# ChrisTho23/DrakeGPT

Measured on AMD Instinct MI355X. Metric: training tokens/sec (fwd+bwd+AdamW), higher is better.
Workload: dtype bf16; 1 GPU; TransformerLM_scaled: V=80 C=384 T=256 heads=6 layers=6 dropout=0.2; fwd+bwd+AdamW; hipGraph=on; batch_per_gpu=64, global_batch=64, seq_len=256, parallelism=dp1, dp_gradient_buckets=1, params=10800464

## Files before the change

### drakegpt_amd/csrc/chain.hip

```cpp
#include "common.h"
#include <stdlib.h>

typedef __attribute__((address_space(1))) const void* gptr_t;
typedef __attribute__((address_space(3))) void* lptr_t;

#define CH_C 384
#define CH_ROWS 64
#define CH_STAGE_B 24576
#define CH_STAGE_A 4096
#define CH_STAGE (CH_STAGE_B + CH_STAGE_A)
#define CH_NST 4
#define CH_ARES (CH_NST * CH_STAGE)
#define CH_KS (CH_C / 32)

struct ChainP {
    const char* o;
    const float* x;
    const char* wproj; const float* bproj;
    float* x1;
    const float* ln2w; const float* ln2b; float* mean2; float* rstd2; bf16_t* h2;
    const char* w1; const float* b1; bf16_t* f; unsigned char* bits;
    const char* w2; const float* b2;
    float* x2; bf16_t* x2b;
    const float* ln1w; const float* ln1b; float* mean1; float* rstd1; bf16_t* h1;
// ... 482 lines not shown
            }
        }
        stamp(12);
        if (HAS_QKV) {
            for (int c = 0; c < 3; ++c) {
                piece(KS, false, c < 2, MODE == 0 && c == 0);
                stamp(13 + 2 * c);
                if (p.dbg == 4 || p.dbg == 5) continue;
                const int lo = opaque_lane(), fr = lo & 15, fg = lo >> 4, col_l = wn * 96 + (fg & 1) * 16 + (fg >> 1) * 8;
#pragma unroll
                for (int q = 0; q < 3; ++q) {
                    const int col = c * C + col_l + 32 * q;
#pragma unroll
                    for (int i = 0; i < 2; ++i) {
                        const int64_t row = row0 + wm * 32 + i * 16 + fr;
                        float v[8];
                        take(i, q, v);
                        bf16x8 o;
#pragma unroll
                        for (int e = 0; e < 8; ++e) o[e] = (bf16_t)v[e];
                        if (p.dbg != 6) *(bf16x8*)(p.qkv + row0 * (3 * C) + mad24(wm * 32 + i * 16 + fr, 3 * C, col)) = o;
                    }
                }
                stamp(14 + 2 * c);
            }
        }
        stamp(19);
        __builtin_amdgcn_s_barrier();
        stamp(20);
    }
}

struct PackOne { const unsigned short* src; unsigned short* dst; int N, K; int64_t ld; };
__global__ __launch_bounds__(256) void pack_chain_kernel(const int64_t* __restrict__ desc, int n_desc, PackOne one) {
    const unsigned short* src = one.src;
    unsigned short* dst = one.dst;
    int K = one.K;
    int64_t ld = one.ld;
    int k = blockIdx.x;
    if (desc) {
        int d = 0;
        for (int i = 1; i < n_desc; ++i)
            if ((int64_t)blockIdx.x >= desc[i * 6 + 4]) d = i;
        const int64_t* D = desc + d * 6;
        src = (const unsigned short*)D[0]; dst = (unsigned short*)D[1]; K = (int)D[3]; ld = D[5];
        k = (int)((int64_t)blockIdx.x - D[4]);
    }
    const int KT = K / 32, c = k / KT, t = k % KT;
    if (!(KT & 1)) {
        const int half = t & 1, t0 = t - half;
        const int64_t k0 = k - half;
#pragma unroll
        for (int u = 0; u < 6; ++u) {
            const int idx = threadIdx.x + 256 * u, line = 96 * half + (idx >> 4), hi = (idx >> 3) & 1, j = idx & 7;
            const int slot = (hi * 4 + (j & 3)) ^ (line & 7);
            const int row = c * 384 + line + 192 * hi, col = t0 * 32 + 8 * j;
            *(u32x4*)(dst + ((k0 + (j >> 2)) * 1536 + line * 8 + slot) * 8) = *(const u32x4*)(src + (int64_t)row * ld + col);
        }
        return;
    }
#pragma unroll
    for (int u = 0; u < 6; ++u) {
        const int idx = threadIdx.x + 256 * u, line = idx >> 3, slot = idx & 7, ls = slot ^ (line & 7);
        const int row = c * 384 + line + 192 * (ls >> 2), col = t * 32 + 8 * (ls & 3);
        *(u32x4*)(dst + ((int64_t)k * 1536 + idx) * 8) = *(const u32x4*)(src + (int64_t)row * ld + col);
    }
}

extern "C" int dg_pack_chain_weights(const void* w, int64_t ld, void* packed, int N, int K, void* stream) {
    if (!w || !packed || N <= 0 || K <= 0 || N % 384 || K % 32 || ld < K || ld % 8 || !dg_aligned16(w) || !dg_aligned16(packed)) return DG_ERR_ARG;
    PackOne one{(const unsigned short*)w, (unsigned short*)packed, N, K, ld};
    hipLaunchKernelGGL(pack_chain_kernel, dim3((N / 384) * (K / 32)), dim3(256), 0, (hipStream_t)stream, (const int64_t*)nullptr, 0, one);
    DG_LAUNCH_CHECK();
    return DG_OK;
}

extern "C" int dg_pack_chain_weights_batched(const int64_t* desc, int n_desc, int total_stages, void* stream) {
    if (!desc || n_desc <= 0 || total_stages <= 0) return DG_ERR_ARG;
    PackOne one{nullptr, nullptr, 0, 0, 0};
    hipLaunchKernelGGL(pack_chain_kernel, dim3(total_stages), dim3(256), 0, (hipStream_t)stream, desc, n_desc, one);
    DG_LAUNCH_CHECK();
    return DG_OK;
}

__global__ __launch_bounds__(256) void l2_warm_kernel(const char* __restrict__ p, int64_t n_lines, float* __restrict__ sink) {
    const int j = (int)blockIdx.x >> 3, per = (int)gridDim.x >> 3;
    float acc = 0.f;
    for (int64_t i = (int64_t)j * 256 + threadIdx.x; i < n_lines; i += (int64_t)per * 256) acc += *(const float*)(p + i * 128);
    if (acc == 123.456f && sink) sink[0] = acc;
}

extern "C" int dg_l2_warm(const void* p, int64_t bytes, void* stream) {
    if (!p || bytes <= 0 || (((uintptr_t)p) & 127)) return DG_ERR_ARG;
    hipLaunchKernelGGL(l2_warm_kernel, dim3(256), dim3(256), 0, (hipStream_t)stream, (const char*)p, bytes / 128, (float*)nullptr);
    DG_LAUNCH_CHECK();
    return DG_OK;
}

static int ch_num_cus() {
    static const int v = [] {
        int dev = 0, n = 256;
        if (hipGetDevice(&dev) == hipSuccess) {
            int x = 0;
            if (hipDeviceGetAttribute(&x, hipDeviceAttributeMultiprocessorCount, dev) == hipSuccess && x > 0) n = x;
        }
        return n;
    }();
    return v;
}

extern "C" int dg_block_chain_supported(int M, int C) { return M > 0 && M % CH_ROWS == 0 && C == CH_C; }

static unsigned long long* g_chain_stamps = nullptr;
// ... 45 lines not shown
```

### drakegpt_amd/csrc/elementwise.hip

```cpp
#include "common.h"

__global__ void state_advance_kernel(uint32_t* st) { st[2] += 1u; }

extern "C" int dg_state_advance(uint32_t* rng_state, void* stream) {
    if (!rng_state) return DG_ERR_ARG;
    hipLaunchKernelGGL(state_advance_kernel, dim3(1), dim3(1), 0, (hipStream_t)stream, rng_state);
    DG_LAUNCH_CHECK();
    return DG_OK;
}

__global__ void batch_gather_kernel(const int64_t* __restrict__ corpus, int64_t n_corpus,
                                    const int64_t* __restrict__ off, int64_t* __restrict__ x,
                                    int64_t* __restrict__ y, int B, int T) {
    int64_t i = (int64_t)blockIdx.x * blockDim.x + threadIdx.x;
    if (i >= (int64_t)B * T) return;
    int b = (int)(i / T), t = (int)(i % T);
    int64_t o = off[b] + t;
    int64_t o1 = o + 1;
    if (o < 0) o = 0; if (o >= n_corpus) o = n_corpus - 1;
    if (o1 < 0) o1 = 0; if (o1 >= n_corpus) o1 = n_corpus - 1;
    x[i] = corpus[o];
    y[i] = corpus[o1];
}

extern "C" int dg_batch_gather(const int64_t* corpus, int64_t n_corpus, const int64_t* offsets,
                               int64_t* x, int64_t* y, int B, int T, void* stream) {
    if (!corpus || !offsets || !x || !y || B <= 0 || T <= 0 || n_corpus < 2) return DG_ERR_ARG;
    int64_t n = (int64_t)B * T;
    hipLaunchKernelGGL(batch_gather_kernel, dim3((unsigned)((n + 255) / 256)), dim3(256), 0,
                       (hipStream_t)stream, corpus, n_corpus, offsets, x, y, B, T);
    DG_LAUNCH_CHECK();
    return DG_OK;
}

struct BatchSrc {
    const int64_t* corpus; int64_t n_corpus; const int64_t* offsets; const uint32_t* step_state; const uint32_t* ctl;
    int64_t* x_ids; int64_t* y_ids; int B;
};
template <int VEC, bool GATHER = false>
__global__ void embed_fwd_kernel(const int64_t* __restrict__ idx, const float* __restrict__ tok,
                                 const float* __restrict__ pos, float* __restrict__ x,
                                 int64_t M, int T, int C, int V, bf16_t* __restrict__ onehot, int64_t ld_onehot, BatchSrc bs) {
    const int cv = C / VEC;
    int64_t total = M * cv;
    const int64_t* off = nullptr;
    if (GATHER) {
        uint32_t row = 0;
        if (bs.ctl) {
            const uint32_t n_rows = bs.ctl[1];
            row = bs.step_state[2] - bs.ctl[0];
            if (row >= n_rows) row = n_rows ? n_rows - 1 : 0;
        }
        off = bs.offsets + (int64_t)row * bs.B;
    }
    (void)total;
    const int lane = threadIdx.x & 63;
    const int64_t wave0 = ((int64_t)blockIdx.x * blockDim.x + threadIdx.x) >> 6, nwaves = ((int64_t)gridDim.x * blockDim.x) >> 6;
    for (int64_t m = wave0; m < M; m += nwaves) {
        const uint32_t mu = (uint32_t)__builtin_amdgcn_readfirstlane((int)m);
        const uint32_t bq = mu / (uint32_t)T;
        const int t = (int)(mu - bq * (uint32_t)T);
        int64_t v;
        if (GATHER) {
            int64_t o = off[bq] + t, o1 = o + 1;
            if (o < 0) o = 0; if (o >= bs.n_corpus) o = bs.n_corpus - 1;
            if (o1 < 0) o1 = 0; if (o1 >= bs.n_corpus) o1 = bs.n_corpus - 1;
            v = bs.corpus[o];
            if (lane == 0) { bs.x_ids[m] = v; bs.y_ids[m] = bs.corpus[o1]; }
        } else {
            v = idx[m];
        }
        v = v < 0 ? 0 : (v >= V ? V - 1 : v);
      for (int j = lane; j < cv; j += 64) {
        const int c = j * VEC;
        if (onehot) {
            if (VEC == 4 && j * 8 < ld_onehot) {
                bf16x8 o;
#pragma unroll
                for (int e = 0; e < 8; ++e) o[e] = (bf16_t)((int64_t)(j * 8 + e) == v ? 1.f : 0.f);
                *(bf16x8*)(onehot + m * ld_onehot + j * 8) = o;
            }
        }
        if (VEC == 4) {
            f32x4 a = *(const f32x4*)(tok + v * C + c);
            if (pos) a += *(const f32x4*)(pos + (int64_t)t * C + c);
            *(f32x4*)(x + m * C + c) = a;
        } else {
            float a = tok[v * C + c];
            if (pos) a += pos[(int64_t)t * C + c];
            x[m * C + c] = a;
        }
      }
    }
}

extern "C" int dg_embed_fwd(const int64_t* idx, const float* tok, const float* pos, float* x,
                            int B, int T, int C, int V, void* onehot, int64_t ld_onehot, void* stream) {
    if (!idx || !tok || !x || B <= 0 || T <= 0 || C <= 0 || V <= 0) return DG_ERR_ARG;
    if (onehot && (C % 4 || ld_onehot % 8 || ld_onehot < V || (int64_t)(C / 4) * 8 < ld_onehot || !dg_aligned16(onehot))) return DG_ERR_ARG;
    int64_t M = (int64_t)B * T;
    bool vec = (C % 4 == 0) && dg_aligned16(tok) && dg_aligned16(x) && (!pos || dg_aligned16(pos));
    int64_t total = vec ? M * (C / 4) : M * C;
    unsigned grid = (unsigned)((total + 255) / 256);
    if (grid > 4096) grid = 4096;
    if (vec)
        hipLaunchKernelGGL(embed_fwd_kernel<4>, dim3(grid), dim3(256), 0, (hipStream_t)stream, idx, tok, pos, x, M, T, C, V, (bf16_t*)onehot, ld_onehot, BatchSrc{});
    else {
        if (onehot) return DG_ERR_ALIGN;
        hipLaunchKernelGGL(embed_fwd_kernel<1>, dim3(grid), dim3(256), 0, (hipStream_t)stream, idx, tok, pos, x, M, T, C, V, (bf16_t*)nullptr, (int64_t)0, BatchSrc{});
    }
    DG_LAUNCH_CHECK();
    return DG_OK;
}

extern "C" int dg_batch_embed_fwd(const int64_t* corpus, int64_t n_corpus, const int64_t* offsets, const uint32_t* step_state,
                                  const uint32_t* ctl, int64_t* x_ids, int64_t* y_ids, const float* tok, const float* pos, float* x,
                                  int B, int T, int C, int V, void* onehot, int64_t ld_onehot, void* stream) {
    if (!corpus || !offsets || !x_ids || !y_ids || !tok || !x || B <= 0 || T <= 0 || C <= 0 || V <= 0 || n_corpus < 2) return DG_ERR_ARG;
    if ((ctl != nullptr) != (step_state != nullptr)) return DG_ERR_ARG;
    if (onehot && (C % 4 || ld_onehot % 8 || ld_onehot < V || (int64_t)(C / 4) * 8 < ld_onehot || !dg_aligned16(onehot))) return DG_ERR_ARG;
    int64_t M = (int64_t)B * T;
    bool vec = (C % 4 == 0) && dg_aligned16(tok) && dg_aligned16(x) && (!pos || dg_aligned16(pos));
    int64_t total = vec ? M * (C / 4) : M * C;
    unsigned grid = (unsigned)((total + 255) / 256);
    if (grid > 4096) grid = 4096;
    const BatchSrc bs{corpus, n_corpus, offsets, step_state, ctl, x_ids, y_ids, B};
    if (vec)
        hipLaunchKernelGGL((embed_fwd_kernel<4, true>), dim3(grid), dim3(256), 0, (hipStream_t)stream, (const int64_t*)nullptr, tok, pos, x, M, T, C, V, (bf16_t*)onehot, ld_onehot, bs);
    else {
        if (onehot) return DG_ERR_ALIGN;
        hipLaunchKernelGGL((embed_fwd_kernel<1, true>), dim3(grid), dim3(256), 0, (hipStream_t)stream, (const int64_t*)nullptr, tok, pos, x, M, T, C, V, (bf16_t*)nullptr, (int64_t)0, bs);
    }
    DG_LAUNCH_CHECK();
    return DG_OK;
}

__global__ void embed_window_kernel(const int64_t* __restrict__ ids, int64_t ld_ids, const uint32_t* __restrict__ state,
                                    const float* __restrict__ tok, const float* __restrict__ pos, float* __restrict__ x,
                                    int B, int Tw, int C, int V, int mode) {
    const int64_t L = (int64_t)state[2];
    if (L < 1 || L > ld_ids || (mode == 0 ? L > Tw : L < Tw)) return;
    const int rows_per_b = mode == 0 ? 1 : Tw;
    const int lane = threadIdx.x & 63;
    const int64_t wave0 = ((int64_t)blockIdx.x * blockDim.x + threadIdx.x) >> 6, nwaves = ((int64_t)gridDim.x * blockDim.x) >> 6;
    const int64_t Mrows = (int64_t)B * rows_per_b;
    for (int64_t m = wave0; m < Mrows; m += nwaves) {
        const int b = (int)(m / rows_per_b), i = (int)(m % rows_per_b);
        const int64_t col = mode == 0 ? L - 1 : L - Tw + i;
        const int t = mode == 0 ? (int)(L - 1) : i;
        int64_t v = ids[(int64_t)b * ld_ids + col];
        v = v < 0 ? 0 : (v >= V ? V - 1 : v);
        for (int c = lane; c < C; c += 64) x[m * C + c] = tok[v * C + c] + pos[(int64_t)t * C + c];
    }
}

extern "C" int dg_embed_window(const int64_t* ids, int64_t ld_ids, const uint32_t* state, const float* tok, const float* pos,
                               float* x, int B, int Tw, int C, int V, int mode, void* stream) {
    if (!ids || !state || !tok || !pos || !x || ld_ids <= 0 || B <= 0 || Tw <= 0 || C <= 0 || V <= 0 || (mode != 0 && mode != 1))
// ... 8 lines not shown

__global__ void zero_f32_kernel(float* __restrict__ p, int64_t n) {
    const int64_t n4 = n / 4;
    for (int64_t i = (int64_t)blockIdx.x * blockDim.x + threadIdx.x; i < n4; i += (int64_t)gridDim.x * blockDim.x)
        ((f32x4*)p)[i] = (f32x4){0.f, 0.f, 0.f, 0.f};
    for (int64_t i = n4 * 4 + (int64_t)blockIdx.x * blockDim.x + threadIdx.x; i < n; i += (int64_t)gridDim.x * blockDim.x) p[i] = 0.f;
}

template <typename TX>
__global__ void embed_bwd_tok_kernel(const int64_t* __restrict__ idx, const TX* __restrict__ dx,
                                     float* __restrict__ dtok, int64_t M, int C, int V) {
    int64_t total = M * C;
    for (int64_t i = (int64_t)blockIdx.x * blockDim.x + threadIdx.x; i < total;
         i += (int64_t)gridDim.x * blockDim.x) {
        int64_t m = i / C;
        int c = (int)(i % C);
        int64_t v = idx[m];
        v = v < 0 ? 0 : (v >= V ? V - 1 : v);
        atomicAdd(dtok + v * C + c, (float)dx[i]);
    }
}
template <typename TX>
__global__ __launch_bounds__(256) void embed_bwd_pos_kernel(const TX* __restrict__ dx, float* __restrict__ dpos,
                                                            int B, int T, int C) {
    __shared__ f32x4 red[4][64];
    const int64_t tc = (int64_t)T * C;
    const int lane = threadIdx.x & 63, g = threadIdx.x >> 6;
    const int64_t i = ((int64_t)blockIdx.x * 64 + lane) * 4;
    const bool vec = (tc % 4 == 0);
    f32x4 s = {0.f, 0.f, 0.f, 0.f};
    if (i < tc) {
        if (vec) {
            typedef TX TX4 __attribute__((ext_vector_type(4)));
            for (int b = g; b < B; b += 4) {
                const TX4 t = *(const TX4*)(dx + (int64_t)b * tc + i);
                s += (f32x4){(float)t[0], (float)t[1], (float)t[2], (float)t[3]};
            }
        } else {
            for (int b = g; b < B; b += 4)
#pragma unroll
                for (int e = 0; e < 4; ++e)
                    if (i + e < tc) s[e] += (float)dx[(int64_t)b * tc + i + e];
        }
    }
    red[g][lane] = s;
    __syncthreads();
    if (g == 0 && i < tc) {
        const f32x4 t = (red[0][lane] + red[1][lane]) + (red[2][lane] + red[3][lane]);
#pragma unroll
        for (int e = 0; e < 4; ++e)
            if (i + e < tc) dpos[i + e] = t[e];
    }
}
extern "C" int dg_embed_bwd(const int64_t* idx, const void* dx_v, int dx_dtype, float* dtok, float* dpos,
                            int B, int T, int C, int V, void* stream) {
    if (dx_dtype != DG_F32 && dx_dtype != DG_BF16) return DG_ERR_DTYPE;
    const float* dx = (const float*)dx_v;
    if (!idx || !dx || (!dtok && !dpos) || B <= 0 || T <= 0 || C <= 0 || V <= 0) return DG_ERR_ARG;
    hipStream_t s = (hipStream_t)stream;
    int64_t M = (int64_t)B * T;
    if (dtok) {
        const int64_t nz = (int64_t)V * C;
        if (!dg_aligned16(dtok)) return DG_ERR_ALIGN;
        unsigned zgrid = (unsigned)((nz / 4 + 255) / 256);
        if (zgrid < 1) zgrid = 1; if (zgrid > 4096) zgrid = 4096;
        hipLaunchKernelGGL(zero_f32_kernel, dim3(zgrid), dim3(256), 0, s, dtok, nz);
        DG_LAUNCH_CHECK();
        int64_t total = M * C;
// ... 74 lines not shown
    else if (dtype == DG_F32)
        hipLaunchKernelGGL(transpose_cast_kernel<float>, grid, dim3(256), 0, (hipStream_t)stream, in, ldi, (float*)out, ldo, R, Cc);
    else
        return DG_ERR_DTYPE;
    DG_LAUNCH_CHECK();
    return DG_OK;
}

template <typename TI, typename TO>
__global__ void transpose_cast_batched_kernel(const int64_t* __restrict__ desc, int n_desc) {
    __shared__ float tile[64][65];
    int d = 0;
    for (int i = 1; i < n_desc; ++i)
        if ((int64_t)blockIdx.x >= desc[i * 8 + 6]) d = i;
    const int64_t* D = desc + d * 8;
    const TI* in = (const TI*)D[0];
    TO* out = (TO*)D[1];
    const int64_t ldi = D[2], ldo = D[3];
    const int R = (int)D[4], Cc = (int)D[5];
    const int local = (int)((int64_t)blockIdx.x - D[6]), tiles_x = (int)D[7];
    const int r0 = (local / tiles_x) * 64, c0 = (local % tiles_x) * 64;
    const int tx = threadIdx.x & 63, ty = threadIdx.x >> 6;
    for (int i = ty; i < 64; i += 4) {
        int r = r0 + i, c = c0 + tx;
        tile[i][tx] = (r < R && c < Cc) ? to_f32<TI>(in[(int64_t)r * ldi + c]) : 0.f;
    }
    __syncthreads();
    for (int i = ty; i < 64; i += 4) {
        int c = c0 + i, r = r0 + tx;
        if (c < Cc && r < ldo) out[(int64_t)c * ldo + r] = from_f32<TO>(tile[tx][i]);
    }
}

__global__ __launch_bounds__(256) void transpose_bf16_batched_kernel(const int64_t* __restrict__ desc, int n_desc) {
    constexpr int PITCH = 68;
    __shared__ __attribute__((aligned(16))) unsigned short tile[64 * PITCH];
    int d = 0;
    for (int i = 1; i < n_desc; ++i)
        if ((int64_t)blockIdx.x >= desc[i * 8 + 6]) d = i;
    const int64_t* D = desc + d * 8;
    const unsigned short* in = (const unsigned short*)D[0];
    unsigned short* out = (unsigned short*)D[1];
    const int64_t ldi = D[2], ldo = D[3];
    const int R = (int)D[4], Cc = (int)D[5];
    const int local = (int)((int64_t)blockIdx.x - D[6]), tiles_x = (int)D[7];
    const int r0 = (local / tiles_x) * 64, c0 = (local % tiles_x) * 64;
    const bool vec = ((ldi | ldo) % 8 == 0) && ((((uintptr_t)in) | ((uintptr_t)out)) % 16 == 0);
#pragma unroll
    for (int pass = 0; pass < 2; ++pass) {
        const int pc = threadIdx.x + 256 * pass, row = pc >> 3, ck = pc & 7;
        const int r = r0 + row, c = c0 + 8 * ck;
        u32x4 v = {0u, 0u, 0u, 0u};
        if (r < R) {
            const unsigned short* src = in + (int64_t)r * ldi + c;
            if (vec && c + 8 <= Cc) v = *(const u32x4*)src;
            else {
                unsigned short e[8];
#pragma unroll
                for (int j = 0; j < 8; ++j) e[j] = (c + j < Cc) ? src[j] : (unsigned short)0;
                v = (u32x4){e[0] | ((uint32_t)e[1] << 16), e[2] | ((uint32_t)e[3] << 16), e[4] | ((uint32_t)e[5] << 16), e[6] | ((uint32_t)e[7] << 16)};
            }
        }
        uint2* dst = (uint2*)(tile + row * PITCH + 8 * ck);
        dst[0] = make_uint2(v[0], v[1]);
        dst[1] = make_uint2(v[2], v[3]);
    }
    __syncthreads();
#pragma unroll
    for (int pass = 0; pass < 2; ++pass) {
        const int pc = threadIdx.x + 256 * pass, oc = (pc & 7) + 8 * (pc >> 6), rk = (pc >> 3) & 7;
        const int c = c0 + oc, r = r0 + 8 * rk;
        if (c >= Cc || r >= ldo) continue;
        unsigned short e[8];
#pragma unroll
        for (int j = 0; j < 8; ++j) e[j] = tile[(8 * rk + j) * PITCH + oc];
        unsigned short* dstp = out + (int64_t)c * ldo + r;
        if (vec && r + 8 <= ldo)
            *(u32x4*)dstp = (u32x4){e[0] | ((uint32_t)e[1] << 16), e[2] | ((uint32_t)e[3] << 16), e[4] | ((uint32_t)e[5] << 16), e[6] | ((uint32_t)e[7] << 16)};
        else {
#pragma unroll
            for (int j = 0; j < 8; ++j)
                if (r + j < ldo) dstp[j] = e[j];
        }
    }
}

__global__ __launch_bounds__(256) void transpose_u8_batched_kernel(const int64_t* __restrict__ desc, int n_desc) {
    constexpr int PITCH = 144;
    __shared__ __attribute__((aligned(16))) unsigned char ta[128 * PITCH], tb[128 * PITCH];
    int d = 0;
    for (int i = 1; i < n_desc; ++i)
        if ((int64_t)blockIdx.x >= desc[i * 8 + 6]) d = i;
    const int64_t* D = desc + d * 8;
    const unsigned char* in = (const unsigned char*)D[0];
    unsigned char* out = (unsigned char*)D[1];
    const int64_t ldi = D[2], ldo = D[3];
    const int R = (int)D[4], Cc = (int)D[5];
    const int local = (int)((int64_t)blockIdx.x - D[6]), tiles_x = (int)D[7];
    const int r0 = (local / tiles_x) * 128, c0 = (local % tiles_x) * 128;
    const bool vec = ((ldi | ldo) % 16 == 0) && ((((uintptr_t)in) | ((uintptr_t)out)) % 16 == 0);
#pragma unroll
    for (int pass = 0; pass < 4; ++pass) {
        const int pc = threadIdx.x + 256 * pass, row = pc >> 3, ck = pc & 7;
        const int r = r0 + row, c = c0 + 16 * ck;
        u32x4 v = {0u, 0u, 0u, 0u};
        if (r < R) {
            const unsigned char* src = in + (int64_t)r * ldi + c;
            if (vec && c + 16 <= Cc) v = *(const u32x4*)src;
            else {
#pragma unroll
                for (int j = 0; j < 16; ++j)
                    if (c + j < Cc) v[j >> 2] |= (uint32_t)src[j] << (8 * (j & 3));
            }
        }
        *(u32x4*)(ta + row * PITCH + 16 * ck) = v;
    }
// ... 12 lines not shown
    }
    __syncthreads();
#pragma unroll
    for (int pass = 0; pass < 4; ++pass) {
        const int pc = threadIdx.x + 256 * pass, row = pc >> 3, ck = pc & 7;
        const int c = c0 + row, r = r0 + 16 * ck;
        if (c >= Cc || r >= ldo) continue;
        const u32x4 v = *(const u32x4*)(tb + row * PITCH + 16 * ck);
        unsigned char* dst = out + (int64_t)c * ldo + r;
        if (vec && r + 16 <= ldo) *(u32x4*)dst = v;
        else {
#pragma unroll
            for (int j = 0; j < 16; ++j)
                if (r + j < ldo) dst[j] = (unsigned char)(v[j >> 2] >> (8 * (j & 3)));
        }
    }
}

extern "C" int dg_transpose_u8_batched(const int64_t* desc, int n_desc, int total_tiles, void* stream) {
    if (!desc || n_desc <= 0 || total_tiles <= 0) return DG_ERR_ARG;
    hipLaunchKernelGGL(transpose_u8_batched_kernel, dim3(total_tiles), dim3(256), 0, (hipStream_t)stream, desc, n_desc);
    DG_LAUNCH_CHECK();
    return DG_OK;
}

extern "C" int dg_transpose_cast_batched(const int64_t* desc, int n_desc, int total_tiles, int in_dtype, int dtype, void* stream) {
    if (!desc || n_desc <= 0 || total_tiles <= 0) return DG_ERR_ARG;
    hipStream_t s = (hipStream_t)stream;
    if (in_dtype == DG_F32 && dtype == DG_BF16)
        hipLaunchKernelGGL((transpose_cast_batched_kernel<float, bf16_t>), dim3(total_tiles), dim3(256), 0, s, desc, n_desc);
    else if (in_dtype == DG_F32 && dtype == DG_F32)
        hipLaunchKernelGGL((transpose_cast_batched_kernel<float, float>), dim3(total_tiles), dim3(256), 0, s, desc, n_desc);
    else if (in_dtype == DG_BF16 && dtype == DG_BF16)
        hipLaunchKernelGGL(transpose_bf16_batched_kernel, dim3(total_tiles), dim3(256), 0, s, desc, n_desc);
    else
        return DG_ERR_DTYPE;
    DG_LAUNCH_CHECK();
    return DG_OK;
}

template <typename TI, typename TO, bool DROP>
__global__ void dropbwd_cast_kernel(const TI* __restrict__ dy, int64_t lddy, TO* __restrict__ g, int64_t ldg,
                                    int M, int N, float inv_keep, uint32_t thr,
                                    const uint32_t* __restrict__ rng_state, uint32_t site,
                                    const float* __restrict__ relu_mask, int64_t ldmask,
                                    float* __restrict__ part, int64_t part_stride, int rows_per) {
    __shared__ float red[4][256];
    const int lane = threadIdx.x & 63, ty = threadIdx.x >> 6;
    const int c = blockIdx.y * 256 + lane * 4;
    const int m_begin = blockIdx.x * rows_per;
    int m_end = m_begin + rows_per; if (m_end > M) m_end = M;
    uint32_t key = 0;
    if (DROP) key = dg_site_key_dev(rng_state, site);
    float acc[4] = {0.f, 0.f, 0.f, 0.f};
    const bool full = (c + 3 < N);
    const bool vec_in = (lddy % 4 == 0) && ((((uintptr_t)dy) % (4 * sizeof(TI))) == 0);
    const bool vec_out = g && (ldg % 4 == 0) && ((((uintptr_t)g) % (4 * sizeof(TO))) == 0);
#pragma unroll 4
    for (int m = m_begin + ty; m < m_end; m += 4) {
        float v[4];
        if (full && vec_in) {
            typedef TI TI4 __attribute__((ext_vector_type(4)));
            const TI4 t = *(const TI4*)(dy + (int64_t)m * lddy + c);
#pragma unroll
            for (int j = 0; j < 4; ++j) v[j] = to_f32<TI>(t[j]);
        } else if (full) {
#pragma unroll
// ... 194 lines not shown
    if (dtype == DG_BF16)
        hipLaunchKernelGGL((dropbwd_cast_kernel<bf16_t, float, false>), grid, block, 0, s, (const bf16_t*)A, lda, (float*)nullptr, (int64_t)0, M, N, 1.f, 0u, (const uint32_t*)nullptr, 0u, (const float*)nullptr, (int64_t)0, part, part_stride, rows_per);
    else if (dtype == DG_F32)
        hipLaunchKernelGGL((dropbwd_cast_kernel<float, float, false>), grid, block, 0, s, (const float*)A, lda, (float*)nullptr, (int64_t)0, M, N, 1.f, 0u, (const uint32_t*)nullptr, 0u, (const float*)nullptr, (int64_t)0, part, part_stride, rows_per);
    else return DG_ERR_DTYPE;
    DG_LAUNCH_CHECK();
    return DG_OK;
}

__global__ void reduce_partials_kernel(const float* __restrict__ part, int64_t stride, int n_partials,
                                       float* __restrict__ out, int64_t n, int vec_ok) {
    int64_t gs = (int64_t)gridDim.x * blockDim.x;
    if (vec_ok) {
        int64_t n4 = n / 4;
        for (int64_t i = (int64_t)blockIdx.x * blockDim.x + threadIdx.x; i < n4; i += gs) {
            f32x4 s = ((const f32x4*)part)[i];
            for (int g = 1; g < n_partials; ++g) s += *(const f32x4*)(part + (int64_t)g * stride + i * 4);
            ((f32x4*)out)[i] = s;
        }
        for (int64_t i = n4 * 4 + (int64_t)blockIdx.x * blockDim.x + threadIdx.x; i < n; i += gs) {
            float s = part[i];
            for (int g = 1; g < n_partials; ++g) s += part[(int64_t)g * stride + i];
            out[i] = s;
        }
    } else {
        for (int64_t i = (int64_t)blockIdx.x * blockDim.x + threadIdx.x; i < n; i += gs) {
            float s = part[i];
            for (int g = 1; g < n_partials; ++g) s += part[(int64_t)g * stride + i];
            out[i] = s;
        }
    }
}

__global__ __launch_bounds__(1024) void reduce_partials_tall_kernel(const float* __restrict__ part, int64_t stride, int n_partials,
                                                                    float* __restrict__ out, int64_t n4) {
    __shared__ f32x4 red[16][64];
    const int c = threadIdx.x & 63, r = threadIdx.x >> 6;
    const int64_t i = (int64_t)blockIdx.x * 64 + c;
    f32x4 s0 = {0.f, 0.f, 0.f, 0.f}, s1 = s0;
    if (i < n4) {
        int g = r;
        for (; g + 16 < n_partials; g += 32) {
            s0 += *(const f32x4*)(part + (int64_t)g * stride + i * 4);
            s1 += *(const f32x4*)(part + (int64_t)(g + 16) * stride + i * 4);
        }
        if (g < n_partials) s0 += *(const f32x4*)(part + (int64_t)g * stride + i * 4);
    }
    red[r][c] = s0 + s1;
    __syncthreads();
    if (r == 0 && i < n4) {
        f32x4 t = red[0][c];
#pragma unroll
        for (int k = 1; k < 16; ++k) t += red[k][c];
        ((f32x4*)out)[i] = t;
    }
}

extern "C" int dg_reduce_partials(const float* partials, int64_t stride, int n_partials,
                                  float* out, int64_t n, void* stream) {
    if (!partials || !out || n_partials <= 0 || n < 0) return DG_ERR_ARG;
    if (n == 0) return DG_OK;
    int vec_ok = dg_aligned16(partials) && dg_aligned16(out) && (stride % 4 == 0);
    if (vec_ok && n_partials >= 32 && n % 4 == 0 && n / 4 < (int64_t)n_partials * 4096) {
        const int64_t n4 = n / 4;
        hipLaunchKernelGGL(reduce_partials_tall_kernel, dim3((unsigned)((n4 + 63) / 64)), dim3(1024), 0, (hipStream_t)stream,
                           partials, stride, n_partials, out, n4);
        DG_LAUNCH_CHECK();
        return DG_OK;
    }
    int64_t work = vec_ok ? (n + 3) / 4 : n;
    unsigned grid = (unsigned)((work + 255) / 256);
    if (grid > 4096) grid = 4096;
    hipLaunchKernelGGL(reduce_partials_kernel, dim3(grid), dim3(256), 0, (hipStream_t)stream, partials, stride, n_partials, out, n, vec_ok);
    DG_LAUNCH_CHECK();
    return DG_OK;
}

__global__ void reduce_sum_kernel(const float* __restrict__ x, int64_t n, float scale, float* __restrict__ out) {
    __shared__ float red[16];
    float s = 0.f;
    for (int64_t i = threadIdx.x; i < n; i += 1024) s += x[i];
    s = wave_sum(s);
    if ((threadIdx.x & 63) == 0) red[threadIdx.x >> 6] = s;
    __syncthreads();
    if (threadIdx.x < 64) {
        float t = threadIdx.x < 16 ? red[threadIdx.x] : 0.f;
        t = wave_sum(t);
        if (threadIdx.x == 0) out[0] = t * scale;
    }
}

extern "C" int dg_reduce_sum(const float* x, int64_t n, float scale, float* out, void* stream) {
    if (!x || !out || n <= 0) return DG_ERR_ARG;
    hipLaunchKernelGGL(reduce_sum_kernel, dim3(1), dim3(1024), 0, (hipStream_t)stream, x, n, scale, out);
    DG_LAUNCH_CHECK();
    return DG_OK;
}

// ... 283 lines not shown
```

Baseline: 7.227 million tokens/s.

## Persistent prefetching pack/transpose kernels, batched embedding rows, unrolled reductions

Turns the weight-pack and batched bf16 transpose kernels into persistent grids that loop over stages or tiles. Each iteration prefetches the next item's global loads while storing the current one, and the descriptor lookup now uses a wave ballot instead of a serial scan. The embedding forward kernel processes four rows per wave so the gather loads are batched, the bias-grad column reduction gets 16/8-way unrolled loads, and the tall partial-reduction kernel is reshaped to 256 threads with 16 columns and deeper unrolling. The aim is to hide memory latency and cut per-block overhead in small memory-bound kernels, at the cost of more registers and more complex indexing.

```diff
diff --git a/drakegpt_amd/csrc/chain.hip b/drakegpt_amd/csrc/chain.hip
--- a/drakegpt_amd/csrc/chain.hip
+++ b/drakegpt_amd/csrc/chain.hip
@@ -538,21 +538,27 @@
 }
 
 struct PackOne { const unsigned short* src; unsigned short* dst; int N, K; int64_t ld; };
-__global__ __launch_bounds__(256) void pack_chain_kernel(const int64_t* __restrict__ desc, int n_desc, PackOne one) {
-    const unsigned short* src = one.src;
-    unsigned short* dst = one.dst;
-    int K = one.K;
-    int64_t ld = one.ld;
-    int k = blockIdx.x;
+typedef __attribute__((address_space(1))) unsigned short g_u16;
+typedef __attribute__((address_space(1))) u32x4 g_u32x4;
+struct PackStage { const g_u16* src; g_u16* dst; int64_t ld; int KT, k; };
+__device__ __forceinline__ PackStage pack_locate(const int64_t* __restrict__ desc, int n_desc, const PackOne& one, int64_t stage, int lane, int64_t first) {
+    PackStage s{(const g_u16*)one.src, (g_u16*)one.dst, one.ld, one.K / 32, (int)stage};
     if (desc) {
-        int d = 0;
-        for (int i = 1; i < n_desc; ++i)
-            if ((int64_t)blockIdx.x >= desc[i * 6 + 4]) d = i;
-        const int64_t* D = desc + d * 6;
-        src = (const unsigned short*)D[0]; dst = (unsigned short*)D[1]; K = (int)D[3]; ld = D[5];
-        k = (int)((int64_t)blockIdx.x - D[4]);
-    }
-    const int KT = K / 32, c = k / KT, t = k % KT;
+        uint64_t m = __ballot(lane >= 1 && lane < n_desc && stage >= first);
+        int d = m ? 63 - __builtin_clzll(m) : 0;
+        for (int base = 64; base < n_desc; base += 64) {
+            const int i = base + lane;
+            m = __ballot(i < n_desc && stage >= desc[(i < n_desc ? i : 0) * 6 + 4]);
+            if (m) d = base + 63 - __builtin_clzll(m);
+        }
+        const int64_t* D = desc + (int64_t)__builtin_amdgcn_readfirstlane(d) * 6;
+        s.src = (const g_u16*)D[0]; s.dst = (g_u16*)D[1]; s.KT = (int)D[3] / 32; s.ld = D[5];
+        s.k = (int)(stage - D[4]);
+    }
+    return s;
+}
+__device__ __forceinline__ void pack_offsets(const PackStage& s, int64_t (&so)[6], int64_t (&po)[6]) {
+    const int k = s.k, KT = s.KT, c = k / KT, t = k % KT;
     if (!(KT & 1)) {
         const int half = t & 1, t0 = t - half;
         const int64_t k0 = k - half;
@@ -561,7 +567,8 @@
             const int idx = threadIdx.x + 256 * u, line = 96 * half + (idx >> 4), hi = (idx >> 3) & 1, j = idx & 7;
             const int slot = (hi * 4 + (j & 3)) ^ (line & 7);
             const int row = c * 384 + line + 192 * hi, col = t0 * 32 + 8 * j;
-            *(u32x4*)(dst + ((k0 + (j >> 2)) * 1536 + line * 8 + slot) * 8) = *(const u32x4*)(src + (int64_t)row * ld + col);
+            so[u] = (int64_t)row * s.ld + col;
+            po[u] = ((k0 + (j >> 2)) * 1536 + line * 8 + slot) * 8;
         }
         return;
     }
@@ -569,14 +576,43 @@
     for (int u = 0; u < 6; ++u) {
         const int idx = threadIdx.x + 256 * u, line = idx >> 3, slot = idx & 7, ls = slot ^ (line & 7);
         const int row = c * 384 + line + 192 * (ls >> 2), col = t * 32 + 8 * (ls & 3);
-        *(u32x4*)(dst + ((int64_t)k * 1536 + idx) * 8) = *(const u32x4*)(src + (int64_t)row * ld + col);
+        so[u] = (int64_t)row * s.ld + col;
+        po[u] = ((int64_t)k * 1536 + idx) * 8;
+    }
+}
+__global__ __launch_bounds__(256) void pack_chain_kernel(const int64_t* __restrict__ desc, int n_desc, PackOne one, int total) {
+    const int lane = threadIdx.x & 63;
+    const int64_t first = (desc && lane < n_desc) ? desc[lane * 6 + 4] : 0;
+    const int64_t s_begin = (int64_t)blockIdx.x * total / gridDim.x, s_end = ((int64_t)blockIdx.x + 1) * total / gridDim.x;
+    if (s_begin >= s_end) return;
+    PackStage cur = pack_locate(desc, n_desc, one, s_begin, lane, first);
+    int64_t so[6], po[6];
+    u32x4 v[6];
+    pack_offsets(cur, so, po);
+#pragma unroll
+    for (int u = 0; u < 6; ++u) v[u] = *(const g_u32x4*)(cur.src + so[u]);
+    for (int64_t st = s_begin; st < s_end; ++st) {
+        u32x4 w[6];
+        int64_t qo[6];
+        g_u16* dst = cur.dst;
+#pragma unroll
+        for (int u = 0; u < 6; ++u) { w[u] = v[u]; qo[u] = po[u]; }
+        if (st + 1 < s_end) {
+            cur = pack_locate(desc, n_desc, one, st + 1, lane, first);
+            pack_offsets(cur, so, po);
+#pragma unroll
+            for (int u = 0; u < 6; ++u) v[u] = *(const g_u32x4*)(cur.src + so[u]);
+        }
+#pragma unroll
+        for (int u = 0; u < 6; ++u) *(g_u32x4*)(dst + qo[u]) = w[u];
     }
 }
 
 extern "C" int dg_pack_chain_weights(const void* w, int64_t ld, void* packed, int N, int K, void* stream) {
     if (!w || !packed || N <= 0 || K <= 0 || N % 384 || K % 32 || ld < K || ld % 8 || !dg_aligned16(w) || !dg_aligned16(packed)) return DG_ERR_ARG;
     PackOne one{(const unsigned short*)w, (unsigned short*)packed, N, K, ld};
-    hipLaunchKernelGGL(pack_chain_kernel, dim3((N / 384) * (K / 32)), dim3(256), 0, (hipStream_t)stream, (const int64_t*)nullptr, 0, one);
+    const int total = (N / 384) * (K / 32);
+    hipLaunchKernelGGL(pack_chain_kernel, dim3(total < 512 ? total : 512), dim3(256), 0, (hipStream_t)stream, (const int64_t*)nullptr, 0, one, total);
     DG_LAUNCH_CHECK();
     return DG_OK;
 }
@@ -584,7 +620,7 @@
 extern "C" int dg_pack_chain_weights_batched(const int64_t* desc, int n_desc, int total_stages, void* stream) {
     if (!desc || n_desc <= 0 || total_stages <= 0) return DG_ERR_ARG;
     PackOne one{nullptr, nullptr, 0, 0, 0};
-    hipLaunchKernelGGL(pack_chain_kernel, dim3(total_stages), dim3(256), 0, (hipStream_t)stream, desc, n_desc, one);
+    hipLaunchKernelGGL(pack_chain_kernel, dim3(total_stages < 512 ? total_stages : 512), dim3(256), 0, (hipStream_t)stream, desc, n_desc, one, total_stages);
     DG_LAUNCH_CHECK();
     return DG_OK;
 }
diff --git a/drakegpt_amd/csrc/elementwise.hip b/drakegpt_amd/csrc/elementwise.hip
--- a/drakegpt_amd/csrc/elementwise.hip
+++ b/drakegpt_amd/csrc/elementwise.hip
@@ -37,6 +37,7 @@
     const int64_t* corpus; int64_t n_corpus; const int64_t* offsets; const uint32_t* step_state; const uint32_t* ctl;
     int64_t* x_ids; int64_t* y_ids; int B;
 };
+constexpr int EMBED_ROWS = 4;
 template <int VEC, bool GATHER = false>
 __global__ void embed_fwd_kernel(const int64_t* __restrict__ idx, const float* __restrict__ tok,
                                  const float* __restrict__ pos, float* __restrict__ x,
@@ -56,39 +57,61 @@
     (void)total;
     const int lane = threadIdx.x & 63;
     const int64_t wave0 = ((int64_t)blockIdx.x * blockDim.x + threadIdx.x) >> 6, nwaves = ((int64_t)gridDim.x * blockDim.x) >> 6;
-    for (int64_t m = wave0; m < M; m += nwaves) {
-        const uint32_t mu = (uint32_t)__builtin_amdgcn_readfirstlane((int)m);
-        const uint32_t bq = mu / (uint32_t)T;
-        const int t = (int)(mu - bq * (uint32_t)T);
-        int64_t v;
-        if (GATHER) {
-            int64_t o = off[bq] + t, o1 = o + 1;
-            if (o < 0) o = 0; if (o >= bs.n_corpus) o = bs.n_corpus - 1;
-            if (o1 < 0) o1 = 0; if (o1 >= bs.n_corpus) o1 = bs.n_corpus - 1;
-            v = bs.corpus[o];
-            if (lane == 0) { bs.x_ids[m] = v; bs.y_ids[m] = bs.corpus[o1]; }
-        } else {
-            v = idx[m];
-        }
-        v = v < 0 ? 0 : (v >= V ? V - 1 : v);
+    for (int64_t m0 = wave0 * EMBED_ROWS; m0 < M; m0 += nwaves * EMBED_ROWS) {
+        const uint32_t mu0 = (uint32_t)__builtin_amdgcn_readfirstlane((int)m0);
+        const int nr = M - m0 < EMBED_ROWS ? (int)(M - m0) : EMBED_ROWS;
+        int64_t vraw[EMBED_ROWS], y[EMBED_ROWS];
+        int vu[EMBED_ROWS], t[EMBED_ROWS];
+#pragma unroll
+        for (int k = 0; k < EMBED_ROWS; ++k) {
+            const uint32_t mu = mu0 + (uint32_t)(k < nr ? k : 0);
+            const uint32_t bq = mu / (uint32_t)T;
+            t[k] = (int)(mu - bq * (uint32_t)T);
+            y[k] = 0;
+            if (GATHER) {
+                int64_t o = off[bq] + t[k], o1 = o + 1;
+                if (o < 0) o = 0; if (o >= bs.n_corpus) o = bs.n_corpus - 1;
+                if (o1 < 0) o1 = 0; if (o1 >= bs.n_corpus) o1 = bs.n_corpus - 1;
+                vraw[k] = bs.corpus[o];
+                y[k] = bs.corpus[o1];
+            } else {
+                vraw[k] = idx[mu];
+            }
+        }
+#pragma unroll
+        for (int k = 0; k < EMBED_ROWS; ++k) {
+            if (GATHER && lane == 0 && k < nr) { bs.x_ids[m0 + k] = vraw[k]; bs.y_ids[m0 + k] = y[k]; }
+            const int64_t v = vraw[k] < 0 ? 0 : (vraw[k] >= V ? V - 1 : vraw[k]);
+            vu[k] = __builtin_amdgcn_readfirstlane((int)v);
+        }
       for (int j = lane; j < cv; j += 64) {
         const int c = j * VEC;
-        if (onehot) {
-            if (VEC == 4 && j * 8 < ld_onehot) {
-                bf16x8 o;
-#pragma unroll
-                for (int e = 0; e < 8; ++e) o[e] = (bf16_t)((int64_t)(j * 8 + e) == v ? 1.f : 0.f);
-                *(bf16x8*)(onehot + m * ld_onehot + j * 8) = o;
-            }
-        }
-        if (VEC == 4) {
-            f32x4 a = *(const f32x4*)(tok + v * C + c);
-            if (pos) a += *(const f32x4*)(pos + (int64_t)t * C + c);
-            *(f32x4*)(x + m * C + c) = a;
-        } else {
-            float a = tok[v * C + c];
-            if (pos) a += pos[(int64_t)t * C + c];
-            x[m * C + c] = a;
+        f32x4 a4[EMBED_ROWS];
+        float a1[EMBED_ROWS];
+#pragma unroll
+        for (int k = 0; k < EMBED_ROWS; ++k) {
+            if (VEC == 4) {
+                a4[k] = *(const f32x4*)(tok + (int64_t)vu[k] * C + c);
+                if (pos) a4[k] += *(const f32x4*)(pos + (int64_t)t[k] * C + c);
+            } else {
+                a1[k] = tok[(int64_t)vu[k] * C + c];
+                if (pos) a1[k] += pos[(int64_t)t[k] * C + c];
+            }
+        }
+#pragma unroll
+        for (int k = 0; k < EMBED_ROWS; ++k) {
+            if (k >= nr) continue;
+            const int64_t m = m0 + k;
+            if (onehot) {
+                if (VEC == 4 && j * 8 < ld_onehot) {
+                    bf16x8 o;
+#pragma unroll
+                    for (int e = 0; e < 8; ++e) o[e] = (bf16_t)((j * 8 + e) == vu[k] ? 1.f : 0.f);
+                    *(bf16x8*)(onehot + m * ld_onehot + j * 8) = o;
+                }
+            }
+            if (VEC == 4) *(f32x4*)(x + m * C + c) = a4[k];
+            else x[m * C + c] = a1[k];
         }
       }
     }
@@ -100,9 +123,8 @@
     if (onehot && (C % 4 || ld_onehot % 8 || ld_onehot < V || (int64_t)(C / 4) * 8 < ld_onehot || !dg_aligned16(onehot))) return DG_ERR_ARG;
     int64_t M = (int64_t)B * T;
     bool vec = (C % 4 == 0) && dg_aligned16(tok) && dg_aligned16(x) && (!pos || dg_aligned16(pos));
-    int64_t total = vec ? M * (C / 4) : M * C;
-    unsigned grid = (unsigned)((total + 255) / 256);
-    if (grid > 4096) grid = 4096;
+    int64_t grid64 = (M + 4 * EMBED_ROWS - 1) / (4 * EMBED_ROWS);
+    unsigned grid = grid64 > 4096 ? 4096u : (unsigned)grid64;
     if (vec)
         hipLaunchKernelGGL(embed_fwd_kernel<4>, dim3(grid), dim3(256), 0, (hipStream_t)stream, idx, tok, pos, x, M, T, C, V, (bf16_t*)onehot, ld_onehot, BatchSrc{});
     else {
@@ -121,9 +143,8 @@
     if (onehot && (C % 4 || ld_onehot % 8 || ld_onehot < V || (int64_t)(C / 4) * 8 < ld_onehot || !dg_aligned16(onehot))) return DG_ERR_ARG;
     int64_t M = (int64_t)B * T;
     bool vec = (C % 4 == 0) && dg_aligned16(tok) && dg_aligned16(x) && (!pos || dg_aligned16(pos));
-    int64_t total = vec ? M * (C / 4) : M * C;
-    unsigned grid = (unsigned)((total + 255) / 256);
-    if (grid > 4096) grid = 4096;
+    int64_t grid64 = (M + 4 * EMBED_ROWS - 1) / (4 * EMBED_ROWS);
+    unsigned grid = grid64 > 4096 ? 4096u : (unsigned)grid64;
     const BatchSrc bs{corpus, n_corpus, offsets, step_state, ctl, x_ids, y_ids, B};
     if (vec)
         hipLaunchKernelGGL((embed_fwd_kernel<4, true>), dim3(grid), dim3(256), 0, (hipStream_t)stream, (const int64_t*)nullptr, tok, pos, x, M, T, C, V, (bf16_t*)onehot, ld_onehot, bs);
@@ -198,8 +219,25 @@
     if (i < tc) {
         if (vec) {
             typedef TX TX4 __attribute__((ext_vector_type(4)));
-            for (int b = g; b < B; b += 4) {
-                const TX4 t = *(const TX4*)(dx + (int64_t)b * tc + i);
+            const TX* src = dx + (int64_t)g * tc + i;
+            const int64_t step = 4 * tc;
+            int b = g;
+            for (; b + 60 < B; b += 64, src += 16 * step) {
+                TX4 t[16];
+#pragma unroll
+                for (int u = 0; u < 16; ++u) t[u] = *(const TX4*)(src + u * step);
+#pragma unroll
+                for (int u = 0; u < 16; ++u) s += (f32x4){(float)t[u][0], (float)t[u][1], (float)t[u][2], (float)t[u][3]};
+            }
+            for (; b + 28 < B; b += 32, src += 8 * step) {
+                TX4 t[8];
+#pragma unroll
+                for (int u = 0; u < 8; ++u) t[u] = *(const TX4*)(src + u * step);
+#pragma unroll
+                for (int u = 0; u < 8; ++u) s += (f32x4){(float)t[u][0], (float)t[u][1], (float)t[u][2], (float)t[u][3]};
+            }
+            for (; b < B; b += 4, src += step) {
+                const TX4 t = *(const TX4*)src;
                 s += (f32x4){(float)t[0], (float)t[1], (float)t[2], (float)t[3]};
             }
         } else {
@@ -340,56 +378,95 @@
     }
 }
 
-__global__ __launch_bounds__(256) void transpose_bf16_batched_kernel(const int64_t* __restrict__ desc, int n_desc) {
+typedef __attribute__((address_space(1))) unsigned short g_u16;
+typedef __attribute__((address_space(1))) u32x4 g_u32x4;
+struct TrTile { const g_u16* in; g_u16* out; int64_t ldi, ldo; int R, Cc, r0, c0, vec; };
+__device__ __forceinline__ TrTile tr_locate(const int64_t* __restrict__ desc, int n_desc, int64_t tile, int lane, int64_t first_tile) {
+    uint64_t m = __ballot(lane >= 1 && lane < n_desc && tile >= first_tile);
+    int d = m ? 63 - __builtin_clzll(m) : 0;
+    for (int base = 64; base < n_desc; base += 64) {
+        const int i = base + lane;
+        m = __ballot(i < n_desc && tile >= desc[(i < n_desc ? i : 0) * 8 + 6]);
+        if (m) d = base + 63 - __builtin_clzll(m);
+    }
+    const int64_t* D = desc + (int64_t)__builtin_amdgcn_readfirstlane(d) * 8;
+    TrTile t;
+    t.in = (const g_u16*)D[0];
+    t.out = (g_u16*)D[1];
+    t.ldi = D[2]; t.ldo = D[3];
+    t.R = (int)D[4]; t.Cc = (int)D[5];
+    const int local = (int)(tile - D[6]), tiles_x = (int)D[7];
+    t.r0 = (local / tiles_x) * 64; t.c0 = (local % tiles_x) * 64;
+    t.vec = ((t.ldi | t.ldo) % 8 == 0) && ((((uintptr_t)t.in) | ((uintptr_t)t.out)) % 16 == 0);
+    return t;
+}
+__device__ __forceinline__ void tr_load(const TrTile& t, u32x4 (&v)[4]) {
+#pragma unroll
+    for (int pass = 0; pass < 4; ++pass) {
+        const int pc = threadIdx.x + 128 * pass, row = pc >> 3, ck = pc & 7;
+        const int r = t.r0 + row, c = t.c0 + 8 * ck;
+        v[pass] = (u32x4){0u, 0u, 0u, 0u};
+        if (r < t.R) {
+            const g_u16* src = t.in + (int64_t)r * t.ldi + c;
+            if (t.vec && c + 8 <= t.Cc) v[pass] = *(const g_u32x4*)src;
+            else {
+                unsigned short e[8];
+#pragma unroll
+                for (int j = 0; j < 8; ++j) e[j] = (c + j < t.Cc) ? src[j] : (unsigned short)0;
+                v[pass] = (u32x4){e[0] | ((uint32_t)e[1] << 16), e[2] | ((uint32_t)e[3] << 16), e[4] | ((uint32_t)e[5] << 16), e[6] | ((uint32_t)e[7] << 16)};
+            }
+        }
+    }
+}
+__global__ __launch_bounds__(128) void transpose_bf16_batched_kernel(const int64_t* __restrict__ desc, int n_desc, int total_tiles) {
     constexpr int PITCH = 68;
     __shared__ __attribute__((aligned(16))) unsigned short tile[64 * PITCH];
-    int d = 0;
-    for (int i = 1; i < n_desc; ++i)
-        if ((int64_t)blockIdx.x >= desc[i * 8 + 6]) d = i;
-    const int64_t* D = desc + d * 8;
-    const unsigned short* in = (const unsigned short*)D[0];
-    unsigned short* out = (unsigned short*)D[1];
-    const int64_t ldi = D[2], ldo = D[3];
-    const int R = (int)D[4], Cc = (int)D[5];
-    const int local = (int)((int64_t)blockIdx.x - D[6]), tiles_x = (int)D[7];
-    const int r0 = (local / tiles_x) * 64, c0 = (local % tiles_x) * 64;
-    const bool vec = ((ldi | ldo) % 8 == 0) && ((((uintptr_t)in) | ((uintptr_t)out)) % 16 == 0);
-#pragma unroll
-    for (int pass = 0; pass < 2; ++pass) {
-        const int pc = threadIdx.x + 256 * pass, row = pc >> 3, ck = pc & 7;
-        const int r = r0 + row, c = c0 + 8 * ck;
-        u32x4 v = {0u, 0u, 0u, 0u};
-        if (r < R) {
-            const unsigned short* src = in + (int64_t)r * ldi + c;
-            if (vec && c + 8 <= Cc) v = *(const u32x4*)src;
+    const int lane = threadIdx.x & 63;
+    const int64_t first_tile = lane < n_desc ? desc[lane * 8 + 6] : 0;
+    const int64_t t_begin = (int64_t)blockIdx.x * total_tiles / gridDim.x, t_end = ((int64_t)blockIdx.x + 1) * total_tiles / gridDim.x;
+    if (t_begin >= t_end) return;
+    TrTile cur = tr_locate(desc, n_desc, t_begin, lane, first_tile);
+    u32x4 v[4];
+    tr_load(cur, v);
+    for (int64_t ti = t_begin; ti < t_end; ++ti) {
+#pragma unroll
+        for (int pass = 0; pass < 4; ++pass) {
+            const int pc = threadIdx.x + 128 * pass, row = pc >> 3, ck = ((pc & 7) + 2 * (row >> 5)) & 7;
+            uint2* dst = (uint2*)(tile + row * PITCH + 8 * ck);
+            dst[0] = make_uint2(v[pass][0], v[pass][1]);
+            dst[1] = make_uint2(v[pass][2], v[pass][3]);
+        }
+        __syncthreads();
+        TrTile nxt = cur;
+        if (ti + 1 < t_end) {
+            nxt = tr_locate(desc, n_desc, ti + 1, lane, first_tile);
+            tr_load(nxt, v);
+        }
+        const int rk = lane & 7, cq = (lane >> 3) + 8 * (threadIdx.x >> 6);
+        uint32_t lo[8], hi[8];
+#pragma unroll
+        for (int j = 0; j < 8; ++j) {
+            const uint2 q = *(const uint2*)(tile + (8 * rk + j) * PITCH + 4 * ((cq + 4 * (rk >> 2)) & 15));
+            lo[j] = q.x; hi[j] = q.y;
+        }
+#pragma unroll
+        for (int e = 0; e < 4; ++e) {
+            const int c = cur.c0 + 4 * cq + e, r = cur.r0 + 8 * rk;
+            if (c >= cur.Cc || r >= cur.ldo) continue;
+            const uint32_t* w = (e & 2) ? hi : lo;
+            const uint32_t sel = (e & 1) ? 0x07060302u : 0x05040100u;
+            const u32x4 o = {__builtin_amdgcn_perm(w[1], w[0], sel), __builtin_amdgcn_perm(w[3], w[2], sel),
+                             __builtin_amdgcn_perm(w[5], w[4], sel), __builtin_amdgcn_perm(w[7], w[6], sel)};
+            g_u16* dstp = cur.out + (int64_t)c * cur.ldo + r;
+            if (cur.vec && r + 8 <= cur.ldo) *(g_u32x4*)dstp = o;
             else {
-                unsigned short e[8];
-#pragma unroll
-                for (int j = 0; j < 8; ++j) e[j] = (c + j < Cc) ? src[j] : (unsigned short)0;
-                v = (u32x4){e[0] | ((uint32_t)e[1] << 16), e[2] | ((uint32_t)e[3] << 16), e[4] | ((uint32_t)e[5] << 16), e[6] | ((uint32_t)e[7] << 16)};
-            }
-        }
-        uint2* dst = (uint2*)(tile + row * PITCH + 8 * ck);
-        dst[0] = make_uint2(v[0], v[1]);
-        dst[1] = make_uint2(v[2], v[3]);
-    }
-    __syncthreads();
-#pragma unroll
-    for (int pass = 0; pass < 2; ++pass) {
-        const int pc = threadIdx.x + 256 * pass, oc = (pc & 7) + 8 * (pc >> 6), rk = (pc >> 3) & 7;
-        const int c = c0 + oc, r = r0 + 8 * rk;
-        if (c >= Cc || r >= ldo) continue;
-        unsigned short e[8];
-#pragma unroll
-        for (int j = 0; j < 8; ++j) e[j] = tile[(8 * rk + j) * PITCH + oc];
-        unsigned short* dstp = out + (int64_t)c * ldo + r;
-        if (vec && r + 8 <= ldo)
-            *(u32x4*)dstp = (u32x4){e[0] | ((uint32_t)e[1] << 16), e[2] | ((uint32_t)e[3] << 16), e[4] | ((uint32_t)e[5] << 16), e[6] | ((uint32_t)e[7] << 16)};
-        else {
-#pragma unroll
-            for (int j = 0; j < 8; ++j)
-                if (r + j < ldo) dstp[j] = e[j];
-        }
+#pragma unroll
+                for (int j = 0; j < 8; ++j)
+                    if (r + j < cur.ldo) dstp[j] = (unsigned short)(o[j >> 1] >> (16 * (j & 1)));
+            }
+        }
+        __syncthreads();
+        cur = nxt;
     }
 }
 
@@ -468,7 +545,7 @@
     else if (in_dtype == DG_F32 && dtype == DG_F32)
         hipLaunchKernelGGL((transpose_cast_batched_kernel<float, float>), dim3(total_tiles), dim3(256), 0, s, desc, n_desc);
     else if (in_dtype == DG_BF16 && dtype == DG_BF16)
-        hipLaunchKernelGGL(transpose_bf16_batched_kernel, dim3(total_tiles), dim3(256), 0, s, desc, n_desc);
+        hipLaunchKernelGGL(transpose_bf16_batched_kernel, dim3(total_tiles < 2048 ? total_tiles : 2048), dim3(128), 0, s, desc, n_desc, total_tiles);
     else
         return DG_ERR_DTYPE;
     DG_LAUNCH_CHECK();
@@ -729,14 +806,35 @@
     }
 }
 
-__global__ __launch_bounds__(1024) void reduce_partials_tall_kernel(const float* __restrict__ part, int64_t stride, int n_partials,
-                                                                    float* __restrict__ out, int64_t n4) {
-    __shared__ f32x4 red[16][64];
-    const int c = threadIdx.x & 63, r = threadIdx.x >> 6;
-    const int64_t i = (int64_t)blockIdx.x * 64 + c;
+constexpr int TALL_COLS = 16;
+__global__ __launch_bounds__(256) void reduce_partials_tall_kernel(const float* __restrict__ part, int64_t stride, int n_partials,
+                                                                   float* __restrict__ out, int64_t n4) {
+    __shared__ f32x4 red[16][TALL_COLS];
+    const int c = threadIdx.x & (TALL_COLS - 1), r = threadIdx.x / TALL_COLS;
+    const int64_t i = (int64_t)blockIdx.x * TALL_COLS + c;
     f32x4 s0 = {0.f, 0.f, 0.f, 0.f}, s1 = s0;
     if (i < n4) {
         int g = r;
+        for (; g + 240 < n_partials; g += 256) {
+            f32x4 a[8], b[8];
+#pragma unroll
+            for (int u = 0; u < 8; ++u) {
+                a[u] = *(const f32x4*)(part + (int64_t)(g + 32 * u) * stride + i * 4);
+                b[u] = *(const f32x4*)(part + (int64_t)(g + 32 * u + 16) * stride + i * 4);
+            }
+#pragma unroll
+            for (int u = 0; u < 8; ++u) { s0 += a[u]; s1 += b[u]; }
+        }
+        for (; g + 112 < n_partials; g += 128) {
+            f32x4 a[4], b[4];
+#pragma unroll
+            for (int u = 0; u < 4; ++u) {
+                a[u] = *(const f32x4*)(part + (int64_t)(g + 32 * u) * stride + i * 4);
+                b[u] = *(const f32x4*)(part + (int64_t)(g + 32 * u + 16) * stride + i * 4);
+            }
+#pragma unroll
+            for (int u = 0; u < 4; ++u) { s0 += a[u]; s1 += b[u]; }
+        }
         for (; g + 16 < n_partials; g += 32) {
             s0 += *(const f32x4*)(part + (int64_t)g * stride + i * 4);
             s1 += *(const f32x4*)(part + (int64_t)(g + 16) * stride + i * 4);
@@ -760,7 +858,7 @@
     int vec_ok = dg_aligned16(partials) && dg_aligned16(out) && (stride % 4 == 0);
     if (vec_ok && n_partials >= 32 && n % 4 == 0 && n / 4 < (int64_t)n_partials * 4096) {
         const int64_t n4 = n / 4;
-        hipLaunchKernelGGL(reduce_partials_tall_kernel, dim3((unsigned)((n4 + 63) / 64)), dim3(1024), 0, (hipStream_t)stream,
+        hipLaunchKernelGGL(reduce_partials_tall_kernel, dim3((unsigned)((n4 + TALL_COLS - 1) / TALL_COLS)), dim3(256), 0, (hipStream_t)stream,
                            partials, stride, n_partials, out, n4);
         DG_LAUNCH_CHECK();
         return DG_OK;
```

After: 7.285 million tokens/s (median of 6 runs). No clear change (+0.8%).
